# zijinxuxu/PDFNet

Hardware: AMD Instinct MI355X
Metric: train-step images/sec @256x256 RGB-D B=32 (higher is better)
Workload: dtype f32

## Files before the change

### pdfnet_amd/csrc/elementwise.hip

```cpp
#include "common.h"

#define GRID_STRIDE(i, total) for (long i = blockIdx.x * (long)blockDim.x + threadIdx.x; i < (total); i += (long)gridDim.x * blockDim.x)

__global__ void act_fwd_kernel(const float* __restrict__ x, int ldx, float* __restrict__ y, int ldy, int C, long total, int act) {
    GRID_STRIDE(i, total) {
        long r = i / C; int c = (int)(i - r * C);
        float v = x[r * ldx + c];
        y[r * ldy + c] = act == 1 ? fmaxf(v, 0.f) : (v > 0.f ? v : 0.1f * v);
    }
}
PDF_API int pdf_act_fwd(const float* x, int ldx, float* y, int ldy, int C, long R, int act, void* stream) {
    hipStream_t s = (hipStream_t)stream;
    if (R * C <= 0) return 0;
    hipLaunchKernelGGL(act_fwd_kernel, dim3(grid_for(R * C)), dim3(256), 0, s, x, ldx, y, ldy, C, R * C, act);
    PDF_LAUNCH_CHECK();
    return 0;
}

__global__ void act_bwd_kernel(const float* __restrict__ dy, int lddy, const float* __restrict__ y, int ldy,
                               float* __restrict__ dx, int lddx, int C, long total, int act) {
    GRID_STRIDE(i, total) {
        long r = i / C; int c = (int)(i - r * C);
        float g = dy[r * lddy + c];
        bool pos = y[r * ldy + c] > 0.f;
// ... 187 lines not shown
PDF_API int pdf_dropout_add(const float* x, const float* res, float* y, long n, float p, unsigned long long seed,
                            const unsigned long long* step, void* stream) {
    hipStream_t s = (hipStream_t)stream;
    if (n <= 0) return 0;
    hipLaunchKernelGGL(dropout_add_kernel, dim3(grid_for(n)), dim3(256), 0, s, x, res, y, n, p, seed, step);
    PDF_LAUNCH_CHECK();
    return 0;
}

__device__ __forceinline__ int maxpool3s2_first_tap(int oy, int ox) { return (oy == 0 ? 3 : 0) + (ox == 0 ? 1 : 0); }
__global__ void maxpool3s2_fwd_kernel(const float* __restrict__ x, int N, int H, int W, int C, int OH, int OW,
                                      float* __restrict__ y, unsigned char* __restrict__ arg, long total) {
    GRID_STRIDE(i, total) {
        int c = (int)(i % C); long p = i / C;
        int ox = (int)(p % OW); p /= OW;
        int oy = (int)(p % OH); int n = (int)(p / OH);
        float best = -INFINITY; int bi = maxpool3s2_first_tap(oy, ox);
        for (int ky = 0; ky < 3; ++ky) {
            int iy = oy * 2 - 1 + ky;
            if (iy < 0 || iy >= H) continue;
            for (int kx = 0; kx < 3; ++kx) {
                int ix = ox * 2 - 1 + kx;
                if (ix < 0 || ix >= W) continue;
                float v = x[(((long)n * H + iy) * W + ix) * C + c];
                if (v > best || v != v) { best = v; bi = ky * 3 + kx; }
            }
        }
        y[i] = best; arg[i] = (unsigned char)bi;
    }
}
__global__ __launch_bounds__(256) void maxpool3s2_fwd_v4_kernel(const float* __restrict__ x, int N, int H, int W, int C, int OH, int OW,
                                                                 float* __restrict__ y, unsigned char* __restrict__ arg, long total4) {
    const int C4 = C >> 2;
    GRID_STRIDE(i, total4) {
        const int c = (int)(i % C4) * 4; long p = i / C4;
        const int ox = (int)(p % OW); p /= OW;
        const int oy = (int)(p % OH); const int n = (int)(p / OH);
        float4 best = make_float4(-INFINITY, -INFINITY, -INFINITY, -INFINITY);
        int b0 = maxpool3s2_first_tap(oy, ox), b1 = b0, b2 = b0, b3 = b0;
#pragma unroll
        for (int ky = 0; ky < 3; ++ky) {
            const int iy = oy * 2 - 1 + ky;
#pragma unroll
            for (int kx = 0; kx < 3; ++kx) {
                const int ix = ox * 2 - 1 + kx;
                if (iy < 0 || iy >= H || ix < 0 || ix >= W) continue;
                const float4 v = *reinterpret_cast<const float4*>(x + (((long)n * H + iy) * W + ix) * C + c);
                const int t = ky * 3 + kx;
                if (v.x > best.x || v.x != v.x) { best.x = v.x; b0 = t; }
                if (v.y > best.y || v.y != v.y) { best.y = v.y; b1 = t; }
                if (v.z > best.z || v.z != v.z) { best.z = v.z; b2 = t; }
                if (v.w > best.w || v.w != v.w) { best.w = v.w; b3 = t; }
            }
        }
        *reinterpret_cast<float4*>(y + i * 4) = best;
        *reinterpret_cast<uchar4*>(arg + i * 4) = make_uchar4((unsigned char)b0, (unsigned char)b1, (unsigned char)b2, (unsigned char)b3);
    }
}
PDF_API int pdf_maxpool3s2_fwd(const float* x, int N, int H, int W, int C, float* y, unsigned char* arg, void* stream) {
    hipStream_t s = (hipStream_t)stream;
    int OH = (H + 2 - 3) / 2 + 1, OW = (W + 2 - 3) / 2 + 1;
    long total = (long)N * OH * OW * C;
    if (total <= 0) return 0;
    if (C % 4 == 0 && !((reinterpret_cast<uintptr_t>(x) | reinterpret_cast<uintptr_t>(y)) & 15) && !(reinterpret_cast<uintptr_t>(arg) & 3))
        hipLaunchKernelGGL(maxpool3s2_fwd_v4_kernel, dim3(grid_for(total / 4)), dim3(256), 0, s, x, N, H, W, C, OH, OW, y, arg, total / 4);
    else
    hipLaunchKernelGGL(maxpool3s2_fwd_kernel, dim3(grid_for(total)), dim3(256), 0, s, x, N, H, W, C, OH, OW, y, arg, total);
    PDF_LAUNCH_CHECK();
    return 0;
}
__global__ void maxpool3s2_bwd_kernel(const float* __restrict__ dy, const unsigned char* __restrict__ arg, int N, int H, int W, int C,
                                      int OH, int OW, float* __restrict__ dx, long total) {
    GRID_STRIDE(i, total) {
        int c = (int)(i % C); long p = i / C;
        int ox = (int)(p % OW); p /= OW;
        int oy = (int)(p % OH); int n = (int)(p / OH);
        int a = arg[i];
        int iy = oy * 2 - 1 + a / 3, ix = ox * 2 - 1 + a % 3;
        atomicAdd(&dx[(((long)n * H + iy) * W + ix) * C + c], dy[i]);
    }
}
__global__ __launch_bounds__(256) void maxpool3s2_bwd_gather_kernel(const float* __restrict__ dy, const unsigned char* __restrict__ arg, int N, int H, int W, int C,
                                                                     int OH, int OW, float* __restrict__ dx, long total4, int accumulate) {
    const int C4 = C >> 2;
    GRID_STRIDE(i, total4) {
        const int c = (int)(i % C4) * 4; long p = i / C4;
        const int ix = (int)(p % W); p /= W;
        const int iy = (int)(p % H); const int n = (int)(p / H);
        float4 g = accumulate ? *reinterpret_cast<const float4*>(dx + i * 4) : make_float4(0.f, 0.f, 0.f, 0.f);
        for (int oy = iy / 2; oy <= min(OH - 1, (iy + 1) / 2); ++oy) {
            const int ky = iy + 1 - 2 * oy;
            if (ky < 0 || ky > 2) continue;
            for (int ox = ix / 2; ox <= min(OW - 1, (ix + 1) / 2); ++ox) {
                const int kx = ix + 1 - 2 * ox;
                if (kx < 0 || kx > 2) continue;
                const long o = (((long)n * OH + oy) * OW + ox) * C + c;
                const uchar4 a = *reinterpret_cast<const uchar4*>(arg + o);
                const float4 d = *reinterpret_cast<const float4*>(dy + o);
                const unsigned char t = (unsigned char)(ky * 3 + kx);
                if (a.x == t) g.x += d.x;
                if (a.y == t) g.y += d.y;
                if (a.z == t) g.z += d.z;
                if (a.w == t) g.w += d.w;
            }
        }
        *reinterpret_cast<float4*>(dx + i * 4) = g;
    }
}
static int maxpool3s2_bwd(const float* dy, const unsigned char* arg, int N, int H, int W, int C, float* dx, int accumulate, hipStream_t s) {
    int OH = (H + 2 - 3) / 2 + 1, OW = (W + 2 - 3) / 2 + 1;
    long total = (long)N * OH * OW * C;
    if (total <= 0) return 0;
    if (C % 4 == 0 && !((reinterpret_cast<uintptr_t>(dy) | reinterpret_cast<uintptr_t>(dx)) & 15) && !(reinterpret_cast<uintptr_t>(arg) & 3)) {
        const long tin4 = (long)N * H * W * C / 4;
        hipLaunchKernelGGL(maxpool3s2_bwd_gather_kernel, dim3(grid_for(tin4)), dim3(256), 0, s, dy, arg, N, H, W, C, OH, OW, dx, tin4, accumulate);
        PDF_LAUNCH_CHECK();
        return 0;
    }
    hipLaunchKernelGGL(maxpool3s2_bwd_kernel, dim3(grid_for(total)), dim3(256), 0, s, dy, arg, N, H, W, C, OH, OW, dx, total);
    PDF_LAUNCH_CHECK();
    return 0;
}
PDF_API int pdf_maxpool3s2_bwd(const float* dy, const unsigned char* arg, int N, int H, int W, int C, float* dx, void* stream) {
    hipStream_t s = (hipStream_t)stream;
    return maxpool3s2_bwd(dy, arg, N, H, W, C, dx, 0, s);
}
PDF_API int pdf_maxpool3s2_bwd_add(const float* dy, const unsigned char* arg, int N, int H, int W, int C, float* dx, void* stream) {
    hipStream_t s = (hipStream_t)stream;
    return maxpool3s2_bwd(dy, arg, N, H, W, C, dx, 1, s);
}

__device__ __forceinline__ void up2_coords(int o, int in_sz, int out_sz, int& i0, int& i1, float& w1) {
    float src = out_sz > 1 ? (float)o * ((float)(in_sz - 1) / (float)(out_sz - 1)) : 0.f;
    i0 = (int)src;
    if (i0 > in_sz - 1) i0 = in_sz - 1;
    i1 = i0 + 1 < in_sz ? i0 + 1 : i0;
    w1 = src - (float)i0;
}
__global__ void up2_fwd_kernel(const float* __restrict__ x, int N, int H, int W, int C, float* __restrict__ y, long total) {
    const int OH = 2 * H, OW = 2 * W;
    GRID_STRIDE(i, total) {
        int c = (int)(i % C); long p = i / C;
        int ox = (int)(p % OW); p /= OW;
        int oy = (int)(p % OH); int n = (int)(p / OH);
        int y0, y1, x0, x1; float wy, wx;
        up2_coords(oy, H, OH, y0, y1, wy);
        up2_coords(ox, W, OW, x0, x1, wx);
        const float* b = x + (long)n * H * W * C + c;
        float v00 = b[((long)y0 * W + x0) * C], v01 = b[((long)y0 * W + x1) * C];
        float v10 = b[((long)y1 * W + x0) * C], v11 = b[((long)y1 * W + x1) * C];
        y[i] = (1.f - wy) * ((1.f - wx) * v00 + wx * v01) + wy * ((1.f - wx) * v10 + wx * v11);
    }
}
__global__ __launch_bounds__(256) void up2_fwd_v4_kernel(const float* __restrict__ x, int H, int W, int C4, float* __restrict__ y) {
    const int OH = 2 * H, OW = 2 * W;
    const int j = blockIdx.x * 256 + threadIdx.x;
    if (j >= OW * C4) return;
    const int ox = j / C4, c4 = j - ox * C4;
    const int n = blockIdx.y / OH, oy = blockIdx.y - n * OH;
    int y0, y1, x0, x1; float wy, wx;
    up2_coords(oy, H, OH, y0, y1, wy);
    up2_coords(ox, W, OW, x0, x1, wx);
    const float4* b = reinterpret_cast<const float4*>(x) + (long)n * H * W * C4 + c4;
    const float4 v00 = b[((long)y0 * W + x0) * C4], v01 = b[((long)y0 * W + x1) * C4];
    const float4 v10 = b[((long)y1 * W + x0) * C4], v11 = b[((long)y1 * W + x1) * C4];
    const float hy = 1.f - wy, hx = 1.f - wx;
    float4 o;
    o.x = hy * (hx * v00.x + wx * v01.x) + wy * (hx * v10.x + wx * v11.x);
    o.y = hy * (hx * v00.y + wx * v01.y) + wy * (hx * v10.y + wx * v11.y);
    o.z = hy * (hx * v00.z + wx * v01.z) + wy * (hx * v10.z + wx * v11.z);
    o.w = hy * (hx * v00.w + wx * v01.w) + wy * (hx * v10.w + wx * v11.w);
    reinterpret_cast<float4*>(y)[((long)blockIdx.y * OW + ox) * C4 + c4] = o;
}
static bool up2_v4_ok(const void* a, const void* b, int N, int H, int W, int C) {
    return C % 4 == 0 && ((reinterpret_cast<uintptr_t>(a) | reinterpret_cast<uintptr_t>(b)) & 15) == 0 && (long)N * 2 * H < 65536 &&
           (long)2 * W * (C / 4) < (1L << 30);
}
PDF_API int pdf_upsample2x_fwd(const float* x, int N, int H, int W, int C, float* y, void* stream) {
    hipStream_t s = (hipStream_t)stream;
    long total = (long)N * 4 * H * W * C;
    if (total <= 0) return 0;
    if (up2_v4_ok(x, y, N, H, W, C)) {
        hipLaunchKernelGGL(up2_fwd_v4_kernel, dim3(cdiv(2 * W * (C / 4), 256), N * 2 * H), dim3(256), 0, s, x, H, W, C / 4, y);
        PDF_LAUNCH_CHECK();
        return 0;
    }
    hipLaunchKernelGGL(up2_fwd_kernel, dim3(grid_for(total)), dim3(256), 0, s, x, N, H, W, C, y, total);
    PDF_LAUNCH_CHECK();
    return 0;
}
__global__ void up2_bwd_kernel(const float* __restrict__ dy, int N, int H, int W, int C, float* __restrict__ dx, long total) {
    const int OH = 2 * H, OW = 2 * W;
    GRID_STRIDE(i, total) {
        int c = (int)(i % C); long p = i / C;
        int ox = (int)(p % OW); p /= OW;
        int oy = (int)(p % OH); int n = (int)(p / OH);
        int y0, y1, x0, x1; float wy, wx;
        up2_coords(oy, H, OH, y0, y1, wy);
        up2_coords(ox, W, OW, x0, x1, wx);
        float g = dy[i];
        float* b = dx + (long)n * H * W * C + c;
        atomicAdd(&b[((long)y0 * W + x0) * C], g * (1.f - wy) * (1.f - wx));
        atomicAdd(&b[((long)y0 * W + x1) * C], g * (1.f - wy) * wx);
        atomicAdd(&b[((long)y1 * W + x0) * C], g * wy * (1.f - wx));
        atomicAdd(&b[((long)y1 * W + x1) * C], g * wy * wx);
    }
}
__device__ __forceinline__ int up2_touching(int i, int in_sz, int out_sz, int (&o_of)[6], float (&w_of)[6]) {
    int cnt = 0;
    const int lo = max(0, 2 * i - 2), hi = min(out_sz - 1, 2 * i + 4);
    for (int o = lo; o <= hi; ++o) {
        int i0, i1; float w1;
        up2_coords(o, in_sz, out_sz, i0, i1, w1);
        float w = 0.f;
        if (i0 == i) w += 1.f - w1;
        if (i1 == i) w += w1;
        if (w != 0.f && cnt < 6) { o_of[cnt] = o; w_of[cnt] = w; ++cnt; }
    }
    return cnt;
}
__global__ __launch_bounds__(256) void up2_bwd_v4_kernel(const float* __restrict__ dy, int H, int W, int C4, float* __restrict__ dx) {
    const int OH = 2 * H, OW = 2 * W;
    const int j = blockIdx.x * 256 + threadIdx.x;
    if (j >= W * C4) return;
    const int ix = j / C4, c4 = j - ix * C4;
    const int n = blockIdx.y / H, iy = blockIdx.y - n * H;
    int oys[6], oxs[6]; float wys[6], wxs[6];
    const int ny = up2_touching(iy, H, OH, oys, wys), nx = up2_touching(ix, W, OW, oxs, wxs);
    const float4* g = reinterpret_cast<const float4*>(dy) + (long)n * OH * OW * C4 + c4;
    float4 acc = make_float4(0.f, 0.f, 0.f, 0.f);
    for (int a = 0; a < ny; ++a)
        for (int b = 0; b < nx; ++b) {
            const float4 v = g[((long)oys[a] * OW + oxs[b]) * C4];
            const float w = wys[a] * wxs[b];
            acc.x += w * v.x; acc.y += w * v.y; acc.z += w * v.z; acc.w += w * v.w;
        }
    reinterpret_cast<float4*>(dx)[((long)blockIdx.y * W + ix) * C4 + c4] = acc;
}
__global__ __launch_bounds__(256) void up2_bwd_gather_kernel(const float* __restrict__ dy, int H, int W, int C, float* __restrict__ dx) {
    const int OH = 2 * H, OW = 2 * W;
    const int j = blockIdx.x * 256 + threadIdx.x;
    if (j >= W * C) return;
    const int ix = j / C, c = j - ix * C;
    const int n = blockIdx.y / H, iy = blockIdx.y - n * H;
    int oys[6], oxs[6]; float wys[6], wxs[6];
    const int ny = up2_touching(iy, H, OH, oys, wys), nx = up2_touching(ix, W, OW, oxs, wxs);
    const float* g = dy + (long)n * OH * OW * C + c;
    float acc = 0.f;
    for (int a = 0; a < ny; ++a)
        for (int b = 0; b < nx; ++b) acc += wys[a] * wxs[b] * g[((long)oys[a] * OW + oxs[b]) * C];
    dx[((long)blockIdx.y * W + ix) * C + c] = acc;
}
PDF_API int pdf_upsample2x_bwd(const float* dy, int N, int H, int W, int C, float* dx, void* stream) {
    hipStream_t s = (hipStream_t)stream;
    long total = (long)N * 4 * H * W * C;
    if (total <= 0) return 0;
    if (up2_v4_ok(dy, dx, N, H, W, C)) {
        hipLaunchKernelGGL(up2_bwd_v4_kernel, dim3(cdiv(W * (C / 4), 256), N * H), dim3(256), 0, s, dy, H, W, C / 4, dx);
        PDF_LAUNCH_CHECK();
        return 0;
    }
    if ((long)N * H < 65536) {
        hipLaunchKernelGGL(up2_bwd_gather_kernel, dim3(cdiv(W * C, 256), N * H), dim3(256), 0, s, dy, H, W, C, dx);
        PDF_LAUNCH_CHECK();
        return 0;
    }
    { hipError_t e = hipMemsetAsync(dx, 0, (size_t)N * H * W * C * sizeof(float), s); if (e != hipSuccess) return (int)e; }
    hipLaunchKernelGGL(up2_bwd_kernel, dim3(grid_for(total)), dim3(256), 0, s, dy, N, H, W, C, dx, total);
    PDF_LAUNCH_CHECK();
    return 0;
}

__global__ void pad2d_kernel(const float* __restrict__ src, int lds, long R, int C, float* __restrict__ dst, int ldd, long R2, int C2) {
    const long total = R2 * C2;
    for (long i = blockIdx.x * (long)blockDim.x + threadIdx.x; i < total; i += (long)gridDim.x * blockDim.x) {
        const long r = i / C2;
        const int c = (int)(i - r * C2);
        dst[r * ldd + c] = (r < R && c < C) ? src[r * lds + c] : 0.f;
    }
}
PDF_API int pdf_pad2d(const float* src, int lds, long R, int C, float* dst, int ldd, long R2, int C2, void* stream) {
    hipStream_t s = (hipStream_t)stream;
    if (R < 0 || C < 0 || R2 < 0 || C2 < 0 || lds < C || ldd < C2) return PDF_E_BADARG;
    if (R2 == 0 || C2 == 0) return 0;
    hipLaunchKernelGGL(pad2d_kernel, dim3(grid_for(R2 * C2)), dim3(256), 0, s, src, lds, R, C, dst, ldd, R2, C2);
    PDF_LAUNCH_CHECK();
    return 0;
}

__global__ void adam_kernel(float* __restrict__ p, const float* __restrict__ g, float* __restrict__ m, float* __restrict__ v, long n,
                            float lr, float b1, float b2, float eps, const float* __restrict__ corr , float grad_scale) {
    const float bc1 = corr[0], bc2 = corr[1];
    const float step = lr / bc1;
    const float rs2 = 1.f / sqrtf(bc2);
    GRID_STRIDE(i, n) {
        float gv = g[i] * grad_scale;
        float mv = b1 * m[i] + (1.f - b1) * gv;
        float vv = b2 * v[i] + (1.f - b2) * gv * gv;
        m[i] = mv; v[i] = vv;
        p[i] -= step * mv / (sqrtf(vv) * rs2 + eps);
    }
}
PDF_API int pdf_adam_step(float* p, const float* g, float* m, float* v, long n, float lr, float b1, float b2, float eps,
                          const float* corr, float grad_scale, void* stream) {
    hipStream_t s = (hipStream_t)stream;
    if (n <= 0) return 0;
    hipLaunchKernelGGL(adam_kernel, dim3(grid_for(n)), dim3(256), 0, s, p, g, m, v, n, lr, b1, b2, eps, corr, grad_scale);
    PDF_LAUNCH_CHECK();
    return 0;
}


#include <atomic>
#include <mutex>
float* pdf_scratch(long floats) {
    static float* base = nullptr;
    static std::once_flag once;
    static std::atomic<long> next{0};
    std::call_once(once, [] { if (hipMalloc(&base, sizeof(float) * PDF_SCRATCH_RING) != hipSuccess) base = nullptr; });
    floats = (floats + 63) & ~63L;
    if (base == nullptr || floats <= 0 || floats > PDF_SCRATCH_MAX) return nullptr;
    long o = next.fetch_add(floats);
    long start = o % PDF_SCRATCH_RING;
    if (start + floats > PDF_SCRATCH_RING) {
        o = next.fetch_add(floats + (PDF_SCRATCH_RING - start)) + (PDF_SCRATCH_RING - start);
        start = o % PDF_SCRATCH_RING;
        if (start + floats > PDF_SCRATCH_RING) start = 0;
    }
    return base + start;
}
static thread_local PdfCallOpts tl_opts = {};
static thread_local long tl_res_tiles = 0, tl_res_rows = 0;
PDF_API int pdf_set_bf16_operands(const void* op0_bf16, const void* op1_bf16) { tl_opts.op0_bf16 = op0_bf16; tl_opts.op1_bf16 = op1_bf16; return 0; }
PDF_API int pdf_set_bf16_output(void* out_bf16) { tl_opts.out_bf16 = out_bf16; return 0; }
PDF_API int pdf_set_bn_input_bf16(const void* x16) { tl_opts.bn_x_bf16 = x16; return 0; }
PDF_API int pdf_set_stats_output(float* part, long cap_floats) { tl_opts.stats_out = part; tl_opts.stats_cap = cap_floats; return 0; }
PDF_API int pdf_set_bn_tile_stats(const float* part, long tiles, long rows_per_tile) { tl_opts.tile_stats = part; tl_opts.tile_n = tiles; tl_opts.tile_rows = rows_per_tile; return 0; }
PDF_API int pdf_set_input_affine_relu(const float* scale, const float* shift) { tl_opts.in_scale = scale; tl_opts.in_shift = shift; return 0; }
PDF_API long pdf_stats_result_tiles(void) { return tl_res_tiles; }
PDF_API long pdf_stats_result_rows(void) { return tl_res_rows; }
PdfPlainCall::PdfPlainCall() : co(tl_opts) { tl_opts = PdfCallOpts{}; co.stats_tiles = co.stats_rows = 0; tl_res_tiles = tl_res_rows = 0; }
PdfPlainCall::~PdfPlainCall() { tl_res_tiles = co.stats_tiles; tl_res_rows = co.stats_rows; }
PDF_API int pdf_debug_armed_slots(void) {
    const PdfCallOpts& o = tl_opts;
    return (o.op0_bf16 != nullptr) + (o.op1_bf16 != nullptr) + (o.out_bf16 != nullptr) + (o.bn_x_bf16 != nullptr) + (o.stats_out != nullptr) +
           (o.tile_stats != nullptr) + (o.in_scale != nullptr) + (o.in_shift != nullptr) + (o.op1_bf16_t != nullptr);
}
PDF_API int pdf_debug_callopts_size(void) { return (int)sizeof(PdfCallOpts); }
__global__ __launch_bounds__(256) void cast_bf16_kernel(const float* __restrict__ src, unsigned short* __restrict__ dst, long n4) {
    for (long i = blockIdx.x * 256L + threadIdx.x; i < n4; i += (long)gridDim.x * 256) {
        const float4 v = reinterpret_cast<const float4*>(src)[i];
        reinterpret_cast<uint2*>(dst)[i] = uint2{pdf_pk_bf16(v.x, v.y), pdf_pk_bf16(v.z, v.w)};
    }
}
PDF_API int pdf_cast_bf16(const float* src, void* dst, long n, void* stream) {
    hipStream_t s = (hipStream_t)stream;
    if (n <= 0) return 0;
    if (n % 4 != 0) return PDF_E_BADARG;
    hipLaunchKernelGGL(cast_bf16_kernel, dim3(grid_for(n / 4)), dim3(256), 0, s, src, reinterpret_cast<unsigned short*>(dst), n / 4);
    PDF_LAUNCH_CHECK();
    return 0;
}

struct PdfTDesc { long src, dst; int R, T, C, tile0; };
__global__ __launch_bounds__(256) void cast_bf16_t_kernel(const float* __restrict__ src, unsigned short* __restrict__ dst,
                                                          const PdfTDesc* __restrict__ tab, int nl) {
    __shared__ float tile[32][33];
    const int bid = blockIdx.x;
    int lo = 0, hi = nl - 1;
    while (lo < hi) { const int mid = (lo + hi + 1) >> 1; if (tab[mid].tile0 <= bid) lo = mid; else hi = mid - 1; }
    const PdfTDesc d = tab[lo];
    const int tr = (d.R + 31) / 32, tc = (d.C + 31) / 32;
    int t = bid - d.tile0;
    const int tap = t / (tr * tc);
    t -= tap * tr * tc;
    const int r0 = (t / tc) * 32, c0 = (t % tc) * 32;
    const int tx = threadIdx.x & 31, ty = threadIdx.x >> 5;
    const float* sp = src + d.src;
    unsigned short* dp = dst + d.dst;
#pragma unroll
    for (int i = 0; i < 4; ++i) {
        const int r = r0 + ty + 8 * i, c = c0 + tx;
        tile[ty + 8 * i][tx] = (r < d.R && c < d.C) ? sp[((long)r * d.T + tap) * d.C + c] : 0.f;
    }
    __syncthreads();
#pragma unroll
    for (int i = 0; i < 4; ++i) {
        const int c = c0 + ty + 8 * i, r = r0 + tx;
        if (r < d.R && c < d.C) dp[((long)c * d.T + tap) * d.R + r] = (unsigned short)(pdf_pk_bf16(tile[tx][ty + 8 * i], 0.f) & 0xffffu);
    }
}
PDF_API int pdf_cast_bf16_transposed(const float* src, void* dst, const void* table, int nlayers, long total_tiles, void* stream) {
    hipStream_t s = (hipStream_t)stream;
    if (nlayers <= 0 || total_tiles <= 0) return 0;
    if (total_tiles > 0x7fffffffL) return PDF_E_BADARG;
    hipLaunchKernelGGL(cast_bf16_t_kernel, dim3((unsigned)total_tiles), dim3(256), 0, s, src, reinterpret_cast<unsigned short*>(dst),
                       reinterpret_cast<const PdfTDesc*>(table), nlayers);
    PDF_LAUNCH_CHECK();
    return 0;
}

#define PDF_EVENT_RING 1024
static hipEvent_t g_events[PDF_EVENT_RING];
static std::atomic<unsigned> g_event_next{0};
static std::atomic<int> g_events_ready{0};
static int pdf_event_ring(void) {
    if (g_events_ready.load(std::memory_order_acquire)) return 0;
    static std::mutex mu;
    std::lock_guard<std::mutex> lk(mu);
    if (g_events_ready.load(std::memory_order_relaxed)) return 0;
    for (int i = 0; i < PDF_EVENT_RING; ++i)
        if (hipEventCreateWithFlags(&g_events[i], hipEventDisableTiming) != hipSuccess) return PDF_E_WORKSPACE;
    g_events_ready.store(1, std::memory_order_release);
    return 0;
}
PDF_API int pdf_stream_wait(void* waiter_stream, void* signaler_stream) {
// ... 34 lines not shown
```

### pdfnet_amd/csrc/pointops.hip

```cpp
#include "common.h"
#include <cstdlib>
#include <mutex>

template <int NPL>
__global__ __launch_bounds__(256) void knn_ball_group_kernel(
    const float* __restrict__ pts, int ldp, int C, int N, int S, int K, float r2,
    int* __restrict__ idx_out, float* __restrict__ grouped, int ldg) {
    extern __shared__ float smem[];
    float* sx = smem;
    float* sy = sx + N;
    float* sz = sy + N;
    int* sidx = reinterpret_cast<int*>(sz + N);
    const int b = blockIdx.y;
    const int tid = threadIdx.x, lane = tid & 63, wave = tid >> 6;
    const float* cloud = pts + (long)b * N * ldp;
    for (int j = tid; j < N; j += 256) {
        sx[j] = cloud[(long)j * ldp + 0];
        sy[j] = cloud[(long)j * ldp + 1];
        sz[j] = cloud[(long)j * ldp + 2];
    }
    __syncthreads();
    int* widx = sidx + wave * K;
    const uint32_t r2bits = __float_as_uint(r2);
    for (int cc = 0; cc < 4; ++cc) {
// ... 117 lines not shown

PDF_API int pdf_group_bwd(const float* dg, int ldg, const int* idx, float* dpts, int ldd, int C,
                          int Bc, int N, int S, int K, void* stream) {
    hipStream_t s = (hipStream_t)stream;
    long rows = (long)Bc * S;
    hipLaunchKernelGGL(group_bwd_kernel, dim3(grid_for(rows * 64)), dim3(256), 0, s, dg, ldg, idx, dpts, ldd, C, N, S, K, rows);
    PDF_LAUNCH_CHECK();
    return 0;
}

__global__ __launch_bounds__(256) void gather_sub_fwd_kernel(const float* __restrict__ u, int ldu, const float* __restrict__ v, int ldv,
                                                             const int* __restrict__ idx, int N, int S, int K, int C,
                                                             float* __restrict__ y, int ldy, long total ) {
    const int cq = C / 4;
    for (long i = blockIdx.x * (long)blockDim.x + threadIdx.x; i < total; i += (long)gridDim.x * blockDim.x) {
        const long row = i / cq;
        const int c0 = (int)(i - row * cq) * 4;
        const long bs = row / K;
        const long b = bs / S;
        const float4 a = *reinterpret_cast<const float4*>(u + (b * N + idx[row]) * ldu + c0);
        const float4 c = *reinterpret_cast<const float4*>(v + bs * ldv + c0);
        *reinterpret_cast<float4*>(y + row * ldy + c0) = make_float4(a.x - c.x, a.y - c.y, a.z - c.z, a.w - c.w);
    }
}
PDF_API int pdf_gather_sub_fwd(const float* u, int ldu, const float* v, int ldv, const int* idx, int Bc, int N, int S, int K, int C,
                               float* y, int ldy, void* stream) {
    hipStream_t s = (hipStream_t)stream;
    if (C % 4 != 0 || ldu % 4 != 0 || ldv % 4 != 0 || ldy % 4 != 0) return PDF_E_BADARG;
    const long total = (long)Bc * S * K * (C / 4);
    if (total == 0) return 0;
    hipLaunchKernelGGL(gather_sub_fwd_kernel, dim3(grid_for(total)), dim3(256), 0, s, u, ldu, v, ldv, idx, N, S, K, C, y, ldy, total);
    PDF_LAUNCH_CHECK();
    return 0;
}
__global__ __launch_bounds__(256) void gather_sub_bwd_kernel(const float* __restrict__ dy, int lddy, const int* __restrict__ idx,
                                                             float* __restrict__ du, int ldu, float* __restrict__ dv, int ldv,
                                                             int N, int S, int K, int C, long total_rows) {
    const int lane = threadIdx.x & 63;
    const long w0 = (blockIdx.x * (long)blockDim.x + threadIdx.x) >> 6;
    const long nw = ((long)gridDim.x * blockDim.x) >> 6;
    for (long row = w0; row < total_rows; row += nw) {
        const long b = row / S;
        float* base = du + b * N * ldu;
        float cs[4] = {0.f, 0.f, 0.f, 0.f};
        for (int k = 0; k < K; ++k) {
            const int j = idx[row * K + k];
            const float* g = dy + (row * K + k) * lddy;
#pragma unroll
            for (int t = 0; t < 4; ++t) {
                const int c = lane + 64 * t;
                if (c < C) {
                    const float x = g[c];
                    atomicAdd(base + (long)j * ldu + c, x);
                    cs[t] += x;
                }
            }
        }
#pragma unroll
        for (int t = 0; t < 4; ++t) {
            const int c = lane + 64 * t;
            if (c < C) dv[row * ldv + c] = -cs[t];
        }
    }
}
#define INV_NT 1024
#define INV_KR 32
__global__ __launch_bounds__(INV_NT) void invert_index_kernel(const int* __restrict__ idx, int N, int E, int nw, int* __restrict__ start,
                                                              int* __restrict__ list) {
    extern __shared__ int sm[];
    int* cnt = sm;
    int* st = sm + (long)nw * N;
    const int b = blockIdx.x, tid = threadIdx.x, lane = tid & 63, wave = tid >> 6;
    const int* id = idx + (long)b * E;
    int* lst = list + (long)b * E;
    for (int i = tid; i < nw * N; i += INV_NT) cnt[i] = 0;
    __syncthreads();
    const int per = ((E + nw - 1) / nw + 63) & ~63;
    const int e0 = wave * per, e1 = min(E, e0 + per);
    int keys[INV_KR];
#pragma unroll
    for (int r = 0; r < INV_KR; ++r) {
        const int e = e0 + r * 64 + lane;
        keys[r] = (wave < nw && e < e1) ? min(max(id[e], 0), N - 1) : -1;
    }
    auto key_of = [&](int r, int e) { return e < e1 ? min(max(id[e], 0), N - 1) : -1; };
    if (wave < nw) {
#pragma unroll
        for (int r = 0; r < INV_KR; ++r) if (keys[r] >= 0) atomicAdd(&cnt[wave * N + keys[r]], 1);
        for (int eb = e0 + INV_KR * 64; eb < e1; eb += 64) { const int k = key_of(0, eb + lane); if (k >= 0) atomicAdd(&cnt[wave * N + k], 1); }
    }
    __syncthreads();
    for (int n = tid; n < N; n += INV_NT) {
        int run = 0;
        for (int w = 0; w < nw; ++w) { const int c = cnt[w * N + n]; cnt[w * N + n] = run; run += c; }
        st[n] = run;
    }
    __syncthreads();
    if (wave == 0) {
        int run = 0;
        for (int n0 = 0; n0 < N; n0 += 64) {
            const int n = n0 + lane;
            const int c = n < N ? st[n] : 0;
            int inc = c;
#pragma unroll
            for (int o = 1; o < 64; o <<= 1) { const int t = __shfl_up(inc, o, 64); if (lane >= o) inc += t; }
            if (n < N) st[n] = run + inc - c;
            run += __shfl(inc, 63, 64);
        }
        if (lane == 0) st[N] = run;
    }
    __syncthreads();
    for (int n = tid; n <= N; n += INV_NT) start[(long)b * (N + 1) + n] = st[n];
    if (wave >= nw) return;
    int* cur = cnt + wave * N;
    const unsigned long long lt = (1ull << lane) - 1ull;
    const int kbits = 32 - __clz(max(N - 1, 1));
    auto place = [&](int key, int e) {
        unsigned long long same = __ballot(key >= 0);
        for (int i = 0; i < kbits; ++i) {
            const bool bit = (key >> i) & 1;
            const unsigned long long m = __ballot(bit);
            same &= bit ? m : ~m;
        }
        if (key >= 0) {
            const int below = __popcll(same & lt);
            lst[st[key] + cur[key] + below] = e;
            if (below == 0) cur[key] += __popcll(same);
        }
    };
#pragma unroll
    for (int r = 0; r < INV_KR; ++r) {
        if (e0 + r * 64 >= e1) break;
        place(keys[r], e0 + r * 64 + lane);
    }
    for (int eb = e0 + INV_KR * 64; eb < e1; eb += 64) place(key_of(0, eb + lane), eb + lane);
}
PDF_API int pdf_invert_index(const int* idx, int Bc, int N, int E, int* start, int* list, int* tmp, void* stream) {
    hipStream_t s = (hipStream_t)stream;
    (void)tmp;
    if (Bc <= 0 || E <= 0) return 0;
    if (N <= 0) return PDF_E_BADARG;
    const long room = 160 * 1024 / 4 - (N + 1);
    int nw = (int)(room / N);
    if (nw > INV_NT / 64) nw = INV_NT / 64;
    if (nw < 1) return PDF_E_BADARG;
    const size_t lds = ((size_t)nw * N + N + 1) * 4;
    static std::once_flag once;
    std::call_once(once, [] { (void)hipFuncSetAttribute(reinterpret_cast<const void*>(invert_index_kernel), hipFuncAttributeMaxDynamicSharedMemorySize, 160 * 1024); });
    hipLaunchKernelGGL(invert_index_kernel, dim3(Bc), dim3(INV_NT), lds, s, idx, N, E, nw, start, list);
    PDF_LAUNCH_CHECK();
    return 0;
}
template <int CL>
__global__ __launch_bounds__(256) void gather_sub_bwd_du_kernel(const float* __restrict__ dy, int lddy, const int* __restrict__ start,
                                                                const int* __restrict__ list, float* __restrict__ du, int ldu,
                                                                int N, int E, int C, long total_points) {
    constexpr int PPW = 64 / CL;
    const int lane = threadIdx.x & 63, sub = lane / CL;
    const long w0 = (blockIdx.x * (long)blockDim.x + threadIdx.x) >> 6;
    const long nw = ((long)gridDim.x * blockDim.x) >> 6;
    const int c4 = (lane % CL) * 4;
    for (long p0 = w0 * PPW; p0 < total_points; p0 += nw * PPW) {
        const long pt = p0 + sub;
        if (pt >= total_points || c4 >= C) continue;
        const long b = pt / N;
        const int n = (int)(pt - b * N);
        const int* st = start + b * (N + 1);
        const int s0 = st[n], s1 = st[n + 1];
        const int* lst = list + b * E;
        const float* g = dy + b * E * lddy;
        float4 acc = make_float4(0.f, 0.f, 0.f, 0.f);
        int j = s0;
        for (; j + 4 <= s1; j += 4) {
            const float4 x0 = *reinterpret_cast<const float4*>(g + (long)lst[j] * lddy + c4);
            const float4 x1 = *reinterpret_cast<const float4*>(g + (long)lst[j + 1] * lddy + c4);
            const float4 x2 = *reinterpret_cast<const float4*>(g + (long)lst[j + 2] * lddy + c4);
            const float4 x3 = *reinterpret_cast<const float4*>(g + (long)lst[j + 3] * lddy + c4);
            acc.x = ((((acc.x + x0.x) + x1.x) + x2.x) + x3.x); acc.y = ((((acc.y + x0.y) + x1.y) + x2.y) + x3.y);
            acc.z = ((((acc.z + x0.z) + x1.z) + x2.z) + x3.z); acc.w = ((((acc.w + x0.w) + x1.w) + x2.w) + x3.w);
        }
        for (; j < s1; ++j) {
            const float4 x = *reinterpret_cast<const float4*>(g + (long)lst[j] * lddy + c4);
            acc.x += x.x; acc.y += x.y; acc.z += x.z; acc.w += x.w;
        }
        *reinterpret_cast<float4*>(du + pt * ldu + c4) = acc;
    }
}
template <int CL>
__global__ __launch_bounds__(256) void gather_sub_bwd_dv_kernel(const float* __restrict__ dy, int lddy, float* __restrict__ dv, int ldv,
                                                                int K, int C, long total_rows) {
    constexpr int PPW = 64 / CL;
    const int lane = threadIdx.x & 63, sub = lane / CL;
    const long w0 = (blockIdx.x * (long)blockDim.x + threadIdx.x) >> 6;
    const long nw = ((long)gridDim.x * blockDim.x) >> 6;
    const int c4 = (lane % CL) * 4;
    for (long r0 = w0 * PPW; r0 < total_rows; r0 += nw * PPW) {
        const long row = r0 + sub;
        if (row >= total_rows || c4 >= C) continue;
        float4 acc = make_float4(0.f, 0.f, 0.f, 0.f);
        const float* g = dy + row * K * lddy + c4;
#pragma unroll 4
        for (int k = 0; k < K; ++k) {
            const float4 x = *reinterpret_cast<const float4*>(g + (long)k * lddy);
            acc.x += x.x; acc.y += x.y; acc.z += x.z; acc.w += x.w;
        }
        *reinterpret_cast<float4*>(dv + row * ldv + c4) = make_float4(-acc.x, -acc.y, -acc.z, -acc.w);
    }
}
PDF_API int pdf_gather_sub_bwd_sorted(const float* dy, int lddy, const int* start, const int* list, float* du, int ldu, float* dv, int ldv,
                                      int Bc, int N, int S, int K, int C, void* stream) {
    hipStream_t s = (hipStream_t)stream;
    if (C > 256 || C % 4 != 0 || lddy % 4 != 0 || ldu % 4 != 0 || ldv % 4 != 0) return PDF_E_BADARG;
    const long pts = (long)Bc * N, rows = (long)Bc * S;
    if (pts == 0 || rows == 0) return 0;
    if (C <= 64) {
        hipLaunchKernelGGL((gather_sub_bwd_du_kernel<16>), dim3(grid_for(pts * 16)), dim3(256), 0, s, dy, lddy, start, list, du, ldu, N, S * K, C, pts);
        hipLaunchKernelGGL((gather_sub_bwd_dv_kernel<16>), dim3(grid_for(rows * 16)), dim3(256), 0, s, dy, lddy, dv, ldv, K, C, rows);
    } else if (C <= 128) {
        hipLaunchKernelGGL((gather_sub_bwd_du_kernel<32>), dim3(grid_for(pts * 32)), dim3(256), 0, s, dy, lddy, start, list, du, ldu, N, S * K, C, pts);
        hipLaunchKernelGGL((gather_sub_bwd_dv_kernel<32>), dim3(grid_for(rows * 32)), dim3(256), 0, s, dy, lddy, dv, ldv, K, C, rows);
    } else {
        hipLaunchKernelGGL((gather_sub_bwd_du_kernel<64>), dim3(grid_for(pts * 64)), dim3(256), 0, s, dy, lddy, start, list, du, ldu, N, S * K, C, pts);
        hipLaunchKernelGGL((gather_sub_bwd_dv_kernel<64>), dim3(grid_for(rows * 64)), dim3(256), 0, s, dy, lddy, dv, ldv, K, C, rows);
    }
    PDF_LAUNCH_CHECK();
    return 0;
}

PDF_API int pdf_gather_sub_bwd(const float* dy, int lddy, const int* idx, float* du, int ldu, float* dv, int ldv,
                               int Bc, int N, int S, int K, int C, void* stream) {
    hipStream_t s = (hipStream_t)stream;
    if (C > 256) return PDF_E_BADARG;
    const long rows = (long)Bc * S;
    if (rows == 0) return 0;
    hipLaunchKernelGGL(gather_sub_bwd_kernel, dim3(grid_for(rows * 64)), dim3(256), 0, s, dy, lddy, idx, du, ldu, dv, ldv, N, S, K, C, rows);
    PDF_LAUNCH_CHECK();
    return 0;
}

__global__ __launch_bounds__(256) void gather_rows_kernel(const float* __restrict__ feat, int ldf, int C, long HW,
                                                          const long* __restrict__ ind, long ind_bstride, int M, int R, int shift,
                                                          float* __restrict__ out, int ldo, long total) {
    const int lane = threadIdx.x & 63;
    const long w0 = (blockIdx.x * (long)blockDim.x + threadIdx.x) >> 6;
    const long nw = ((long)gridDim.x * blockDim.x) >> 6;
    for (long r = w0; r < total; r += nw) {
        const long b = r / M;
        long i = ind[b * ind_bstride + (r - b * M)];
        if (shift > 0) {
            long y = i / R, x = i - y * R;
            i = (y >> shift) * (R >> shift) + (x >> shift);
        }
        const float* p = feat + (b * HW + i) * ldf;
        float* o = out + r * ldo;
        for (int c = lane; c < ldo; c += 64) o[c] = c < C ? p[c] : 0.f;
    }
}

PDF_API int pdf_gather_rows(const float* feat, int ldf, int C, long HW, const long* ind, long ind_bstride,
                            int B, int M, int R, int shift, float* out, int ldo, void* stream) {
    hipStream_t s = (hipStream_t)stream;
    long total = (long)B * M;
    if (total == 0) return 0;
    hipLaunchKernelGGL(gather_rows_kernel, dim3(grid_for(total * 64)), dim3(256), 0, s, feat, ldf, C, HW, ind, ind_bstride, M, R, shift, out, ldo, total);
    PDF_LAUNCH_CHECK();
    return 0;
}

__global__ __launch_bounds__(256) void scatter_rows_kernel(const float* __restrict__ dout, int ldo, int C, long HW,
                                                           const long* __restrict__ ind, long ind_bstride, int M, int R, int shift,
                                                           float* __restrict__ dfeat, int ldf, long total) {
    const int lane = threadIdx.x & 63;
    const long w0 = (blockIdx.x * (long)blockDim.x + threadIdx.x) >> 6;
    const long nw = ((long)gridDim.x * blockDim.x) >> 6;
    for (long r = w0; r < total; r += nw) {
        const long b = r / M;
        long i = ind[b * ind_bstride + (r - b * M)];
        if (shift > 0) {
            long y = i / R, x = i - y * R;
            i = (y >> shift) * (R >> shift) + (x >> shift);
        }
        float* p = dfeat + (b * HW + i) * ldf;
        const float* o = dout + r * ldo;
        for (int c = lane; c < C; c += 64) atomicAdd(p + c, o[c]);
    }
}

PDF_API int pdf_scatter_rows_add(const float* dout, int ldo, int C, long HW, const long* ind, long ind_bstride,
                                 int B, int M, int R, int shift, float* dfeat, int ldf, void* stream) {
    hipStream_t s = (hipStream_t)stream;
    long total = (long)B * M;
    if (total == 0) return 0;
    hipLaunchKernelGGL(scatter_rows_kernel, dim3(grid_for(total * 64)), dim3(256), 0, s, dout, ldo, C, HW, ind, ind_bstride, M, R, shift, dfeat, ldf, total);
    PDF_LAUNCH_CHECK();
    return 0;
}

__global__ __launch_bounds__(256) void maxk_fwd_kernel(const float* __restrict__ x, int ldx, int C, int K,
                                                       float* __restrict__ y, int ldy, int* __restrict__ arg, long total) {
    for (long i = blockIdx.x * (long)blockDim.x + threadIdx.x; i < total; i += (long)gridDim.x * blockDim.x) {
        const long r = i / C;
        const int c = (int)(i - r * C);
        const float* p = x + r * K * ldx + c;
        float best = p[0];
        int bi = 0;
        for (int k = 1; k < K; ++k) {
            float v = p[(long)k * ldx];
            if (v > best) { best = v; bi = k; }
        }
        y[r * ldy + c] = best;
        arg[r * C + c] = bi;
    }
}

PDF_API int pdf_maxk_fwd(const float* x, int ldx, int C, long R, int K, float* y, int ldy, int* arg, void* stream) {
    hipStream_t s = (hipStream_t)stream;
    long total = R * C;
    if (total == 0) return 0;
    hipLaunchKernelGGL(maxk_fwd_kernel, dim3(grid_for(total)), dim3(256), 0, s, x, ldx, C, K, y, ldy, arg, total);
    PDF_LAUNCH_CHECK();
    return 0;
}

__global__ __launch_bounds__(256) void maxk_bwd_kernel(const float* __restrict__ dy, int ldy, const int* __restrict__ arg,
                                                       int C, int K, float* __restrict__ dx, int ldx, long total) {
    for (long i = blockIdx.x * (long)blockDim.x + threadIdx.x; i < total; i += (long)gridDim.x * blockDim.x) {
        const long rk = i / C;
        const int c = (int)(i - rk * C);
        const long r = rk / K;
        const int k = (int)(rk - r * K);
        dx[rk * ldx + c] = (arg[r * C + c] == k) ? dy[r * ldy + c] : 0.f;
    }
}

PDF_API int pdf_maxk_bwd(const float* dy, int ldy, const int* arg, int C, long R, int K, float* dx, int ldx, void* stream) {
    hipStream_t s = (hipStream_t)stream;
    long total = R * K * C;
    if (total == 0) return 0;
    hipLaunchKernelGGL(maxk_bwd_kernel, dim3(grid_for(total)), dim3(256), 0, s, dy, ldy, arg, C, K, dx, ldx, total);
    PDF_LAUNCH_CHECK();
    return 0;
}

__global__ __launch_bounds__(256) void window_kernel(float* __restrict__ feat, int ldf, int C, int H, int W,
                                                     const long* __restrict__ ind, long ind_bstride, int M, int r,
                                                     float* __restrict__ buf, const float* __restrict__ src, int mode, long total) {
    const int lane = threadIdx.x & 63;
    const int win = 2 * r + 1;
    const long w0 = (blockIdx.x * (long)blockDim.x + threadIdx.x) >> 6;
    const long nw = ((long)gridDim.x * blockDim.x) >> 6;
    for (long p = w0; p < total; p += nw) {
        long q = p;
        const int wx = (int)(q % win); q /= win;
        const int wy = (int)(q % win); q /= win;
        const long b = q / M;
        const long i = ind[b * ind_bstride + (q - b * M)];
        const int y = (int)(i / W) - r + wy, x = (int)(i % W) - r + wx;
        const bool in = y >= 0 && y < H && x >= 0 && x < W;
        float* row = buf + p * C;
        if (mode == 2) {
            const float* s = src + p * C;
            for (int c = lane; c < C; c += 64) row[c] = in ? s[c] : 0.f;
        } else {
            float* f = feat + ((b * H + y) * (long)W + x) * ldf;
            if (mode == 0) { for (int c = lane; c < C; c += 64) row[c] = in ? f[c] : 0.f; }
            else if (in) { for (int c = lane; c < C; c += 64) atomicAdd(f + c, row[c]); }
        }
    }
}

PDF_API int pdf_window_op(float* feat, int ldf, int C, int H, int W, const long* ind, long ind_bstride,
                          int B, int M, int r, float* buf, const float* src, int mode, void* stream) {
    hipStream_t s = (hipStream_t)stream;
    long total = (long)B * M * (2 * r + 1) * (2 * r + 1);
    if (total <= 0) return 0;
    hipLaunchKernelGGL(window_kernel, dim3(grid_for(total * 64)), dim3(256), 0, s, feat, ldf, C, H, W, ind, ind_bstride, M, r, buf, src, mode, total);
    PDF_LAUNCH_CHECK();
// ... 177 lines not shown
```

Baseline: 721.8.

## Tile upsample fwd/bwd across rows and fuse sorted gather-sub backward kernels

```diff
diff --git a/pdfnet_amd/csrc/elementwise.hip b/pdfnet_amd/csrc/elementwise.hip
--- a/pdfnet_amd/csrc/elementwise.hip
+++ b/pdfnet_amd/csrc/elementwise.hip
@@ -363,25 +363,47 @@
         y[i] = (1.f - wy) * ((1.f - wx) * v00 + wx * v01) + wy * ((1.f - wx) * v10 + wx * v11);
     }
 }
+constexpr int UP2_FWD_ROWS = 4;
+__device__ __forceinline__ float4 up2_pick(float4 h0, float4 h1, float4 h2, float4 h3, int k) {
+    float4 t = h0;
+    if (k == 1) t = h1;
+    if (k == 2) t = h2;
+    if (k == 3) t = h3;
+    return t;
+}
 __global__ __launch_bounds__(256) void up2_fwd_v4_kernel(const float* __restrict__ x, int H, int W, int C4, float* __restrict__ y) {
     const int OH = 2 * H, OW = 2 * W;
-    const int j = blockIdx.x * 256 + threadIdx.x;
-    if (j >= OW * C4) return;
-    const int ox = j / C4, c4 = j - ox * C4;
-    const int n = blockIdx.y / OH, oy = blockIdx.y - n * OH;
-    int y0, y1, x0, x1; float wy, wx;
-    up2_coords(oy, H, OH, y0, y1, wy);
+    const int c4 = blockIdx.z * blockDim.x + threadIdx.x, ox = blockIdx.x * blockDim.y + threadIdx.y;
+    if (c4 >= C4 || ox >= OW) return;
+    const int groups = (OH + UP2_FWD_ROWS - 1) / UP2_FWD_ROWS;
+    const int n = blockIdx.y / groups, oy0 = (blockIdx.y - n * groups) * UP2_FWD_ROWS;
+    int x0, x1, a, a1; float wx, wa;
     up2_coords(ox, W, OW, x0, x1, wx);
+    up2_coords(oy0, H, OH, a, a1, wa);
+    const float hx = 1.f - wx;
     const float4* b = reinterpret_cast<const float4*>(x) + (long)n * H * W * C4 + c4;
-    const float4 v00 = b[((long)y0 * W + x0) * C4], v01 = b[((long)y0 * W + x1) * C4];
-    const float4 v10 = b[((long)y1 * W + x0) * C4], v11 = b[((long)y1 * W + x1) * C4];
-    const float hy = 1.f - wy, hx = 1.f - wx;
-    float4 o;
-    o.x = hy * (hx * v00.x + wx * v01.x) + wy * (hx * v10.x + wx * v11.x);
-    o.y = hy * (hx * v00.y + wx * v01.y) + wy * (hx * v10.y + wx * v11.y);
-    o.z = hy * (hx * v00.z + wx * v01.z) + wy * (hx * v10.z + wx * v11.z);
-    o.w = hy * (hx * v00.w + wx * v01.w) + wy * (hx * v10.w + wx * v11.w);
-    reinterpret_cast<float4*>(y)[((long)blockIdx.y * OW + ox) * C4 + c4] = o;
+    float4 h[UP2_FWD_ROWS];
+#pragma unroll
+    for (int k = 0; k < UP2_FWD_ROWS; ++k) {
+        const long row = (long)min(a + k, H - 1) * W;
+        const float4 v0 = b[(row + x0) * C4], v1 = b[(row + x1) * C4];
+        h[k] = make_float4(hx * v0.x + wx * v1.x, hx * v0.y + wx * v1.y, hx * v0.z + wx * v1.z, hx * v0.w + wx * v1.w);
+    }
+    float4* out = reinterpret_cast<float4*>(y) + (((long)n * OH + oy0) * OW + ox) * C4 + c4;
+#pragma unroll
+    for (int r = 0; r < UP2_FWD_ROWS; ++r) {
+        if (oy0 + r >= OH) break;
+        int y0, y1; float wy;
+        up2_coords(oy0 + r, H, OH, y0, y1, wy);
+        const float4 t = up2_pick(h[0], h[1], h[2], h[3], y0 - a), u = up2_pick(h[0], h[1], h[2], h[3], y1 - a);
+        const float hy = 1.f - wy;
+        out[(long)r * OW * C4] = make_float4(hy * t.x + wy * u.x, hy * t.y + wy * u.y, hy * t.z + wy * u.z, hy * t.w + wy * u.w);
+    }
+}
+static dim3 up2_block(int units, int cap) {
+    int bx = 1;
+    while (bx < units && bx < cap) bx *= 2;
+    return dim3(bx, 256 / bx);
 }
 static bool up2_v4_ok(const void* a, const void* b, int N, int H, int W, int C) {
     return C % 4 == 0 && ((reinterpret_cast<uintptr_t>(a) | reinterpret_cast<uintptr_t>(b)) & 15) == 0 && (long)N * 2 * H < 65536 &&
@@ -392,7 +414,8 @@
     long total = (long)N * 4 * H * W * C;
     if (total <= 0) return 0;
     if (up2_v4_ok(x, y, N, H, W, C)) {
-        hipLaunchKernelGGL(up2_fwd_v4_kernel, dim3(cdiv(2 * W * (C / 4), 256), N * 2 * H), dim3(256), 0, s, x, H, W, C / 4, y);
+        const dim3 blk = up2_block(C / 4, 64);
+        hipLaunchKernelGGL(up2_fwd_v4_kernel, dim3(cdiv(2 * W, blk.y), N * cdiv(2 * H, UP2_FWD_ROWS), cdiv(C / 4, blk.x)), blk, 0, s, x, H, W, C / 4, y);
         PDF_LAUNCH_CHECK();
         return 0;
     }
@@ -417,62 +440,105 @@
         atomicAdd(&b[((long)y1 * W + x1) * C], g * wy * wx);
     }
 }
-__device__ __forceinline__ int up2_touching(int i, int in_sz, int out_sz, int (&o_of)[6], float (&w_of)[6]) {
-    int cnt = 0;
-    const int lo = max(0, 2 * i - 2), hi = min(out_sz - 1, 2 * i + 4);
-    for (int o = lo; o <= hi; ++o) {
-        int i0, i1; float w1;
-        up2_coords(o, in_sz, out_sz, i0, i1, w1);
-        float w = 0.f;
-        if (i0 == i) w += 1.f - w1;
-        if (i1 == i) w += w1;
-        if (w != 0.f && cnt < 6) { o_of[cnt] = o; w_of[cnt] = w; ++cnt; }
-    }
-    return cnt;
-}
-__global__ __launch_bounds__(256) void up2_bwd_v4_kernel(const float* __restrict__ dy, int H, int W, int C4, float* __restrict__ dx) {
-    const int OH = 2 * H, OW = 2 * W;
-    const int j = blockIdx.x * 256 + threadIdx.x;
-    if (j >= W * C4) return;
-    const int ix = j / C4, c4 = j - ix * C4;
-    const int n = blockIdx.y / H, iy = blockIdx.y - n * H;
-    int oys[6], oxs[6]; float wys[6], wxs[6];
-    const int ny = up2_touching(iy, H, OH, oys, wys), nx = up2_touching(ix, W, OW, oxs, wxs);
-    const float4* g = reinterpret_cast<const float4*>(dy) + (long)n * OH * OW * C4 + c4;
-    float4 acc = make_float4(0.f, 0.f, 0.f, 0.f);
-    for (int a = 0; a < ny; ++a)
-        for (int b = 0; b < nx; ++b) {
-            const float4 v = g[((long)oys[a] * OW + oxs[b]) * C4];
-            const float w = wys[a] * wxs[b];
-            acc.x += w * v.x; acc.y += w * v.y; acc.z += w * v.z; acc.w += w * v.w;
-        }
-    reinterpret_cast<float4*>(dx)[((long)blockIdx.y * W + ix) * C4 + c4] = acc;
-}
-__global__ __launch_bounds__(256) void up2_bwd_gather_kernel(const float* __restrict__ dy, int H, int W, int C, float* __restrict__ dx) {
-    const int OH = 2 * H, OW = 2 * W;
-    const int j = blockIdx.x * 256 + threadIdx.x;
-    if (j >= W * C) return;
-    const int ix = j / C, c = j - ix * C;
-    const int n = blockIdx.y / H, iy = blockIdx.y - n * H;
-    int oys[6], oxs[6]; float wys[6], wxs[6];
-    const int ny = up2_touching(iy, H, OH, oys, wys), nx = up2_touching(ix, W, OW, oxs, wxs);
-    const float* g = dy + (long)n * OH * OW * C + c;
-    float acc = 0.f;
-    for (int a = 0; a < ny; ++a)
-        for (int b = 0; b < nx; ++b) acc += wys[a] * wxs[b] * g[((long)oys[a] * OW + oxs[b]) * C];
-    dx[((long)blockIdx.y * W + ix) * C + c] = acc;
+constexpr int UP2_BWD_ROWS = 4;
+constexpr int UP2_BWD_ITS = 3;
+__device__ __forceinline__ void up2_fma(float& a, float w, float v) { a += w * v; }
+__device__ __forceinline__ void up2_fma(float4& a, float w, const float4& v) { a.x += w * v.x; a.y += w * v.y; a.z += w * v.z; a.w += w * v.w; }
+__device__ __forceinline__ void up2_clear(float& a) { a = 0.f; }
+__device__ __forceinline__ void up2_clear(float4& a) { a = make_float4(0.f, 0.f, 0.f, 0.f); }
+__device__ __forceinline__ float up2_weight(int i, int i0, int i1, float w1) { return (i0 == i ? 1.f - w1 : 0.f) + (i1 == i ? w1 : 0.f); }
+template <typename V>
+__global__ __launch_bounds__(256) void up2_bwd_gather_kernel(const V* __restrict__ dy, int H, int W, int CU, V* __restrict__ dx) {
+    extern __shared__ float4 up2_smem[];
+    const int OH = 2 * H, OW = 2 * W, bx = blockDim.x, by = blockDim.y, tx = threadIdx.x, ty = threadIdx.y;
+    const int ncmax = 2 * by + 5;
+    V* t = reinterpret_cast<V*>(up2_smem);
+    int* sx0 = reinterpret_cast<int*>(t + UP2_BWD_ROWS * ncmax * bx);
+    float* swx = reinterpret_cast<float*>(sx0 + ncmax);
+    const int strips = (H + UP2_BWD_ROWS - 1) / UP2_BWD_ROWS;
+    const int n = blockIdx.y / strips, iy0 = (blockIdx.y - n * strips) * UP2_BWD_ROWS, ix0 = blockIdx.x * by;
+    const int c = blockIdx.z * bx + tx;
+    const bool cok = c < CU;
+    const int ox_lo = max(0, 2 * ix0 - 2), ncols = min(OW - 1, 2 * (ix0 + by - 1) + 4) - ox_lo + 1;
+    const int oy_lo = max(0, 2 * iy0 - 2), oy_hi = min(OH - 1, 2 * (iy0 + UP2_BWD_ROWS - 1) + 4);
+    for (int col = ty * bx + tx; col < ncols; col += 256) {
+        int x0, x1; float w1;
+        up2_coords(ox_lo + col, W, OW, x0, x1, w1);
+        sx0[col] = x0; swx[col] = w1;
+    }
+    V acc[UP2_BWD_ITS][UP2_BWD_ROWS];
+#pragma unroll
+    for (int it = 0; it < UP2_BWD_ITS; ++it)
+#pragma unroll
+        for (int r = 0; r < UP2_BWD_ROWS; ++r) up2_clear(acc[it][r]);
+    const V* g = dy + ((long)n * OH * OW + ox_lo) * CU + c;
+#pragma unroll 2
+    for (int oy = oy_lo; oy <= oy_hi; ++oy) {
+        int y0, y1; float wy;
+        up2_coords(oy, H, OH, y0, y1, wy);
+        V v[UP2_BWD_ITS];
+#pragma unroll
+        for (int it = 0; it < UP2_BWD_ITS; ++it) {
+            const int col = ty + it * by;
+            if (cok && col < ncols) v[it] = g[((long)oy * OW + col) * CU];
+            else up2_clear(v[it]);
+        }
+#pragma unroll
+        for (int r = 0; r < UP2_BWD_ROWS; ++r) {
+            const float w = up2_weight(iy0 + r, y0, y1, wy);
+            if (w != 0.f) {
+#pragma unroll
+                for (int it = 0; it < UP2_BWD_ITS; ++it) up2_fma(acc[it][r], w, v[it]);
+            }
+        }
+    }
+#pragma unroll
+    for (int it = 0; it < UP2_BWD_ITS; ++it) {
+        const int col = ty + it * by;
+        if (col < ncols) {
+#pragma unroll
+            for (int r = 0; r < UP2_BWD_ROWS; ++r) t[(r * ncmax + col) * bx + tx] = acc[it][r];
+        }
+    }
+    __syncthreads();
+    const int ix = ix0 + ty;
+    if (!cok || ix >= W) return;
+    V out[UP2_BWD_ROWS];
+#pragma unroll
+    for (int r = 0; r < UP2_BWD_ROWS; ++r) up2_clear(out[r]);
+    const int c_hi = min(ncols - 1, 2 * ix + 4 - ox_lo);
+    for (int col = max(0, 2 * ix - 2 - ox_lo); col <= c_hi; ++col) {
+        const int x0 = sx0[col];
+        const float w = up2_weight(ix, x0, min(x0 + 1, W - 1), swx[col]);
+        if (w != 0.f) {
+#pragma unroll
+            for (int r = 0; r < UP2_BWD_ROWS; ++r) up2_fma(out[r], w, t[(r * ncmax + col) * bx + tx]);
+        }
+    }
+    V* o = dx + (((long)n * H + iy0) * W + ix) * CU + c;
+#pragma unroll
+    for (int r = 0; r < UP2_BWD_ROWS; ++r)
+        if (iy0 + r < H) o[(long)r * W * CU] = out[r];
+}
+template <typename V>
+static void up2_bwd_gather(const float* dy, int N, int H, int W, int CU, float* dx, hipStream_t s) {
+    const dim3 blk = up2_block(CU, sizeof(V) == 16 ? 8 : 32);
+    const int ncmax = 2 * blk.y + 5;
+    const size_t lds = (size_t)UP2_BWD_ROWS * ncmax * blk.x * sizeof(V) + ncmax * (sizeof(int) + sizeof(float));
+    hipLaunchKernelGGL(up2_bwd_gather_kernel<V>, dim3(cdiv(W, blk.y), N * cdiv(H, UP2_BWD_ROWS), cdiv(CU, blk.x)), blk, lds, s,
+                       reinterpret_cast<const V*>(dy), H, W, CU, reinterpret_cast<V*>(dx));
 }
 PDF_API int pdf_upsample2x_bwd(const float* dy, int N, int H, int W, int C, float* dx, void* stream) {
     hipStream_t s = (hipStream_t)stream;
     long total = (long)N * 4 * H * W * C;
     if (total <= 0) return 0;
     if (up2_v4_ok(dy, dx, N, H, W, C)) {
-        hipLaunchKernelGGL(up2_bwd_v4_kernel, dim3(cdiv(W * (C / 4), 256), N * H), dim3(256), 0, s, dy, H, W, C / 4, dx);
+        up2_bwd_gather<float4>(dy, N, H, W, C / 4, dx, s);
         PDF_LAUNCH_CHECK();
         return 0;
     }
     if ((long)N * H < 65536) {
-        hipLaunchKernelGGL(up2_bwd_gather_kernel, dim3(cdiv(W * C, 256), N * H), dim3(256), 0, s, dy, H, W, C, dx);
+        up2_bwd_gather<float>(dy, N, H, W, C, dx, s);
         PDF_LAUNCH_CHECK();
         return 0;
     }
diff --git a/pdfnet_amd/csrc/pointops.hip b/pdfnet_amd/csrc/pointops.hip
--- a/pdfnet_amd/csrc/pointops.hip
+++ b/pdfnet_amd/csrc/pointops.hip
@@ -293,60 +293,56 @@
     return 0;
 }
 template <int CL>
-__global__ __launch_bounds__(256) void gather_sub_bwd_du_kernel(const float* __restrict__ dy, int lddy, const int* __restrict__ start,
-                                                                const int* __restrict__ list, float* __restrict__ du, int ldu,
-                                                                int N, int E, int C, long total_points) {
-    constexpr int PPW = 64 / CL;
-    const int lane = threadIdx.x & 63, sub = lane / CL;
-    const long w0 = (blockIdx.x * (long)blockDim.x + threadIdx.x) >> 6;
-    const long nw = ((long)gridDim.x * blockDim.x) >> 6;
-    const int c4 = (lane % CL) * 4;
-    for (long p0 = w0 * PPW; p0 < total_points; p0 += nw * PPW) {
-        const long pt = p0 + sub;
-        if (pt >= total_points || c4 >= C) continue;
-        const long b = pt / N;
-        const int n = (int)(pt - b * N);
+__global__ __launch_bounds__(256) void gather_sub_bwd_sorted_kernel(const float* __restrict__ dy, int lddy, const int* __restrict__ start,
+                                                                    const int* __restrict__ list, float* __restrict__ du, int ldu,
+                                                                    float* __restrict__ dv, int ldv, int Bc, int N, int S, int K, int C, int tasks_du, int tasks) {
+    constexpr int PPW = 64 / CL, RIF = 8;
+    const int lane = threadIdx.x & 63, sub = lane / CL, c4 = (lane % CL) * 4;
+    const long w = (blockIdx.x * (long)blockDim.x + threadIdx.x) >> 6;
+    const long b = w / tasks;
+    const int task = (int)(w - b * tasks);
+    if (b >= Bc || c4 >= C) return;
+    const long E = (long)S * K;
+    const float* g = dy + b * E * lddy + c4;
+    float4 acc = make_float4(0.f, 0.f, 0.f, 0.f);
+    if (task < tasks_du) {
+        const int n = task * PPW + sub;
+        if (n >= N) return;
         const int* st = start + b * (N + 1);
         const int s0 = st[n], s1 = st[n + 1];
         const int* lst = list + b * E;
-        const float* g = dy + b * E * lddy;
-        float4 acc = make_float4(0.f, 0.f, 0.f, 0.f);
-        int j = s0;
-        for (; j + 4 <= s1; j += 4) {
-            const float4 x0 = *reinterpret_cast<const float4*>(g + (long)lst[j] * lddy + c4);
-            const float4 x1 = *reinterpret_cast<const float4*>(g + (long)lst[j + 1] * lddy + c4);
-            const float4 x2 = *reinterpret_cast<const float4*>(g + (long)lst[j + 2] * lddy + c4);
-            const float4 x3 = *reinterpret_cast<const float4*>(g + (long)lst[j + 3] * lddy + c4);
-            acc.x = ((((acc.x + x0.x) + x1.x) + x2.x) + x3.x); acc.y = ((((acc.y + x0.y) + x1.y) + x2.y) + x3.y);
-            acc.z = ((((acc.z + x0.z) + x1.z) + x2.z) + x3.z); acc.w = ((((acc.w + x0.w) + x1.w) + x2.w) + x3.w);
-        }
-        for (; j < s1; ++j) {
-            const float4 x = *reinterpret_cast<const float4*>(g + (long)lst[j] * lddy + c4);
-            acc.x += x.x; acc.y += x.y; acc.z += x.z; acc.w += x.w;
-        }
-        *reinterpret_cast<float4*>(du + pt * ldu + c4) = acc;
-    }
-}
-template <int CL>
-__global__ __launch_bounds__(256) void gather_sub_bwd_dv_kernel(const float* __restrict__ dy, int lddy, float* __restrict__ dv, int ldv,
-                                                                int K, int C, long total_rows) {
-    constexpr int PPW = 64 / CL;
-    const int lane = threadIdx.x & 63, sub = lane / CL;
-    const long w0 = (blockIdx.x * (long)blockDim.x + threadIdx.x) >> 6;
-    const long nw = ((long)gridDim.x * blockDim.x) >> 6;
-    const int c4 = (lane % CL) * 4;
-    for (long r0 = w0 * PPW; r0 < total_rows; r0 += nw * PPW) {
-        const long row = r0 + sub;
-        if (row >= total_rows || c4 >= C) continue;
-        float4 acc = make_float4(0.f, 0.f, 0.f, 0.f);
-        const float* g = dy + row * K * lddy + c4;
-#pragma unroll 4
+        int slot[RIF];
+#pragma unroll
+        for (int r = 0; r < RIF; ++r) slot[r] = s0 < s1 ? lst[min(s0 + r, s1 - 1)] : 0;
+        for (int j = s0; j < s1; j += RIF) {
+            float4 x[RIF];
+#pragma unroll
+            for (int r = 0; r < RIF; ++r) x[r] = *reinterpret_cast<const float4*>(g + (long)slot[r] * lddy);
+#pragma unroll
+            for (int r = 0; r < RIF; ++r) slot[r] = lst[min(j + RIF + r, s1 - 1)];
+#pragma unroll
+            for (int r = 0; r < RIF; ++r)
+                if (j + r < s1) { acc.x += x[r].x; acc.y += x[r].y; acc.z += x[r].z; acc.w += x[r].w; }
+        }
+        *reinterpret_cast<float4*>(du + (b * N + n) * ldu + c4) = acc;
+    } else {
+        const int sc = (task - tasks_du) * PPW + sub;
+        if (sc >= S) return;
+        g += (long)sc * K * lddy;
+#pragma unroll 8
         for (int k = 0; k < K; ++k) {
             const float4 x = *reinterpret_cast<const float4*>(g + (long)k * lddy);
             acc.x += x.x; acc.y += x.y; acc.z += x.z; acc.w += x.w;
         }
-        *reinterpret_cast<float4*>(dv + row * ldv + c4) = make_float4(-acc.x, -acc.y, -acc.z, -acc.w);
-    }
+        *reinterpret_cast<float4*>(dv + (b * S + sc) * ldv + c4) = make_float4(-acc.x, -acc.y, -acc.z, -acc.w);
+    }
+}
+template <int CL>
+static void gather_sub_bwd_sorted(const float* dy, int lddy, const int* start, const int* list, float* du, int ldu, float* dv, int ldv,
+                                  int Bc, int N, int S, int K, int C, hipStream_t s) {
+    const int tasks_du = cdiv(N, 64 / CL), tasks = tasks_du + cdiv(S, 64 / CL);
+    hipLaunchKernelGGL((gather_sub_bwd_sorted_kernel<CL>), dim3(cdiv((long)Bc * tasks, 4)), dim3(256), 0, s, dy, lddy, start, list, du, ldu, dv, ldv,
+                       Bc, N, S, K, C, tasks_du, tasks);
 }
 PDF_API int pdf_gather_sub_bwd_sorted(const float* dy, int lddy, const int* start, const int* list, float* du, int ldu, float* dv, int ldv,
                                       int Bc, int N, int S, int K, int C, void* stream) {
@@ -354,16 +350,9 @@
     if (C > 256 || C % 4 != 0 || lddy % 4 != 0 || ldu % 4 != 0 || ldv % 4 != 0) return PDF_E_BADARG;
     const long pts = (long)Bc * N, rows = (long)Bc * S;
     if (pts == 0 || rows == 0) return 0;
-    if (C <= 64) {
-        hipLaunchKernelGGL((gather_sub_bwd_du_kernel<16>), dim3(grid_for(pts * 16)), dim3(256), 0, s, dy, lddy, start, list, du, ldu, N, S * K, C, pts);
-        hipLaunchKernelGGL((gather_sub_bwd_dv_kernel<16>), dim3(grid_for(rows * 16)), dim3(256), 0, s, dy, lddy, dv, ldv, K, C, rows);
-    } else if (C <= 128) {
-        hipLaunchKernelGGL((gather_sub_bwd_du_kernel<32>), dim3(grid_for(pts * 32)), dim3(256), 0, s, dy, lddy, start, list, du, ldu, N, S * K, C, pts);
-        hipLaunchKernelGGL((gather_sub_bwd_dv_kernel<32>), dim3(grid_for(rows * 32)), dim3(256), 0, s, dy, lddy, dv, ldv, K, C, rows);
-    } else {
-        hipLaunchKernelGGL((gather_sub_bwd_du_kernel<64>), dim3(grid_for(pts * 64)), dim3(256), 0, s, dy, lddy, start, list, du, ldu, N, S * K, C, pts);
-        hipLaunchKernelGGL((gather_sub_bwd_dv_kernel<64>), dim3(grid_for(rows * 64)), dim3(256), 0, s, dy, lddy, dv, ldv, K, C, rows);
-    }
+    if (C <= 64) gather_sub_bwd_sorted<16>(dy, lddy, start, list, du, ldu, dv, ldv, Bc, N, S, K, C, s);
+    else if (C <= 128) gather_sub_bwd_sorted<32>(dy, lddy, start, list, du, ldu, dv, ldv, Bc, N, S, K, C, s);
+    else gather_sub_bwd_sorted<64>(dy, lddy, start, list, du, ldu, dv, ldv, Bc, N, S, K, C, s);
     PDF_LAUNCH_CHECK();
     return 0;
 }
```

Result: no change. 724.4, median of 6 (+0.4%).
